# Lucaskabela/UNAST

Hardware: AMD Instinct MI355X
Metric: mel-frames/sec/node (train step, gen+disc) at B=32,T_mel=800; 1/2/4/8-GPU scaling (higher is better)
Workload: dtype bf16x3

## Files before the change

unast_amd/csrc/loss.hip:

```cpp
#include "common.h"

__global__ __launch_bounds__(256) void speech_loss_fwd_kernel(const float* __restrict__ gold, const float* __restrict__ head, int ldh,
                                                              const float* __restrict__ post, const int* __restrict__ lens, int B, int T, int M,
                                                              float eos_weight, double* __restrict__ ws, float* __restrict__ loss) {
    const int rows = B * T;
    const int mq = M >> 2;
    const size_t total = (size_t)rows * mq;
    float a0 = 0.f, a1 = 0.f, a2 = 0.f;
    for (size_t i = (size_t)blockIdx.x * 256 + threadIdx.x; i < total; i += (size_t)gridDim.x * 256) {
        const int r = (int)(i / mq), c = (int)(i - (size_t)r * mq) * 4;
        const int b = r / T, t = r - b * T;
        const int len = lens[b];
        if (t < len) {
            float4 g = *reinterpret_cast<const float4*>(gold + (size_t)r * M + c);
            float4 p = *reinterpret_cast<const float4*>(head + (size_t)r * ldh + c);
            float4 q = *reinterpret_cast<const float4*>(post + (size_t)r * M + c);
            float d;
            d = g.x - p.x; a0 += d * d; d = g.y - p.y; a0 += d * d; d = g.z - p.z; a0 += d * d; d = g.w - p.w; a0 += d * d;
            d = g.x - q.x; a1 += d * d; d = g.y - q.y; a1 += d * d; d = g.z - q.z; a1 += d * d; d = g.w - q.w; a1 += d * d;
        }
        if (c == 0) {
            const float x = head[(size_t)r * ldh + M];
            const float y = (t == len - 1) ? 1.f : 0.f;
            const float lw = 1.f + (eos_weight - 1.f) * y;
// ... 309 lines not shown
                    const float bb[4] = {b4.x, b4.y, b4.z, b4.w};
                    float gd[4] = {0.f, 0.f, 0.f, 0.f};
                    if (live) { const float4 g4 = *reinterpret_cast<const float4*>(gold + (size_t)m * M + n0); gd[0] = g4.x; gd[1] = g4.y; gd[2] = g4.z; gd[3] = g4.w; }
#pragma unroll
                    for (int r = 0; r < 4; ++r) {
                        const float p = acc[c2][r] + bb[r];
                        hp[r] = p;
                        if (live) { const float d = p - gd[r]; a0 += d * d; dp[r] = km * d; }
                    }
                } else if (n0 == M) {
                    const float x = acc[c2][0] + bias[M];
                    const float y = (tt == len - 1) ? 1.f : 0.f;
                    const float lw = 1.f + (eos_weight - 1.f) * y;
                    hp[0] = x;
                    a2 += (1.f - y) * x + lw * (log1pf(expf(-fabsf(x))) + fmaxf(-x, 0.f));
                    dp[0] = ks * ((1.f - y) - lw * (1.f - 1.f / (1.f + expf(-x))));
                }
                *reinterpret_cast<float4*>(head + (size_t)m * ldh + n0) = hv;
                *reinterpret_cast<float4*>(d_head + (size_t)m * ldh + n0) = dv;
            }
        }
    }
    __shared__ double red[8][2];
    const double d0 = wave_sum_d((double)a0), d2 = wave_sum_d((double)a2);
    if (lane == 0) { red[wave][0] = d0; red[wave][1] = d2; }
    __syncthreads();
    if (t < 2) {
        double v = 0.0;
        for (int w = 0; w < 8; ++w) v += red[w][t];
        atomicAdd(ws + (t == 0 ? 0 : 2), v);
    }
}

__global__ __launch_bounds__(256) void speech_post_loss_kernel(const float* __restrict__ gold, const float* __restrict__ post, const int* __restrict__ lens,
                                                               int B, int T, int M, float gscale, float* __restrict__ d_post, double* __restrict__ ws,
                                                               float* __restrict__ loss) {
    __shared__ float s_denom;
    if (threadIdx.x == 0) {
        double sl = 0.0;
        for (int b = 0; b < B; ++b) sl += (double)lens[b];
        s_denom = (float)(sl * (double)M);
    }
    __syncthreads();
    const float km = 2.f * gscale / s_denom;
    const int rows = B * T, mq = M >> 2;
    const size_t total = (size_t)rows * mq;
    float a1 = 0.f;
    for (size_t i = (size_t)blockIdx.x * 256 + threadIdx.x; i < total; i += (size_t)gridDim.x * 256) {
        const int r = (int)(i / mq), c = (int)(i - (size_t)r * mq) * 4;
        const int b = r / T, t = r - b * T;
        float4 o = make_float4(0.f, 0.f, 0.f, 0.f);
        if (t < lens[b]) {
            const float4 g = *reinterpret_cast<const float4*>(gold + (size_t)r * M + c);
            const float4 q = *reinterpret_cast<const float4*>(post + (size_t)r * M + c);
            const float dx = q.x - g.x, dy = q.y - g.y, dz = q.z - g.z, dw = q.w - g.w;
            a1 += (dx * dx + dy * dy) + (dz * dz + dw * dw);
            o = make_float4(km * dx, km * dy, km * dz, km * dw);
        }
        *reinterpret_cast<float4*>(d_post + (size_t)r * M + c) = o;
    }
    __shared__ double red[4];
    const double d1 = wave_sum_d((double)a1);
    if ((threadIdx.x & 63) == 0) red[threadIdx.x >> 6] = d1;
    __syncthreads();
    if (threadIdx.x == 0) {
        atomicAdd(ws + 1, (red[0] + red[1]) + (red[2] + red[3]));
        __threadfence();
        const unsigned long long arrived = atomicAdd(reinterpret_cast<unsigned long long*>(ws + 3), 1ull) + 1ull;
        if (arrived == gridDim.x) {
            __threadfence();
            const double s0 = atomicAdd(ws + 0, 0.0), s1 = atomicAdd(ws + 1, 0.0), s2 = atomicAdd(ws + 2, 0.0);
            const double denom = (double)s_denom;
            loss[0] = (float)(s0 / denom + s1 / denom + s2 / ((double)B * T));
            ws[0] = 0.0; ws[1] = 0.0; ws[2] = 0.0; reinterpret_cast<unsigned long long*>(ws)[3] = 0ull;
        }
    }
}

__global__ __launch_bounds__(256) void disc_targets_kernel(const int64_t* __restrict__ perm, int n, int B, int flip, float smoothing, float* __restrict__ out) {
    for (int i = threadIdx.x; i < n; i += 256) {
        float y = 1.f - smoothing;
        if (perm[i] >= B) y = 1.f - y;
        if (flip) y = 1.f - y;
        out[i] = y;
    }
}

__global__ __launch_bounds__(256) void bce_logits_kernel(const float* __restrict__ logits, int ldx, const float* __restrict__ targets, int n,
                                                         const float* __restrict__ gscale, float* __restrict__ loss, float* __restrict__ dlogits, int ldd) {
    __shared__ float red[4];
    float a = 0.f;
    const float g = gscale ? gscale[0] : 0.f;
    for (int i = threadIdx.x; i < n; i += 256) {
        const float y = targets[i];
        const float x = logits[(size_t)i * ldx];
// ... 129 lines not shown
    UNAST_REQUIRE(a && out && div != 0.f, "unast_scalar_combine: bad arguments");
    hipLaunchKernelGGL(scalar_combine_kernel, dim3(1), dim3(64), 0, stream, a, b, c, div, out);
    return unast_check_launch("unast_scalar_combine");
}

extern "C" int unast_text_head_loss(const float* X, int ldx, const float* W, const float* bias, const int64_t* gold, int rows, int K, int V,
                                    float eos_weight, float gscale, float* logits, float* dlogits, int ldl, double* ws, float* loss, hipStream_t stream) {
    const int eos_idx = 2, pad_idx = 0;
    UNAST_REQUIRE(X && W && bias && gold && logits && dlogits && ws && loss && rows > 0, "unast_text_head_loss: bad arguments");
    UNAST_REQUIRE(K == 256 && V > 0 && V <= 48 && ldl >= V && ldl <= 48 && (ldl & 3) == 0 && (ldx & 3) == 0, "unast_text_head_loss: built for K = 256, V <= 48, 16-byte row strides (K=%d V=%d ldl=%d)", K, V, ldl);
    UNAST_REQUIRE((((uintptr_t)X | (uintptr_t)W | (uintptr_t)logits | (uintptr_t)dlogits) & 15) == 0, "unast_text_head_loss: operands must be 16-byte aligned");
    hipLaunchKernelGGL(text_head_loss_kernel, dim3((rows + 127) / 128), dim3(512), 0, stream, X, ldx, W, bias, gold, rows, V, eos_idx, eos_weight, pad_idx,
                       gscale, logits, dlogits, ldl, ws, loss);
    return unast_check_launch("unast_text_head_loss");
}

extern "C" int unast_speech_head_loss(const float* X, int ldx, const float* W, const float* bias, const float* gold, const int* lens, int B, int T, int K, int M,
                                      float eos_weight, float gscale, float* head, float* d_head, int ldh, double* ws, hipStream_t stream) {
    UNAST_REQUIRE(X && W && bias && gold && lens && head && d_head && ws && B > 0 && T > 0, "unast_speech_head_loss: bad arguments");
    UNAST_REQUIRE(K == 256 && M > 0 && (M & 3) == 0 && M + 1 <= 96 && ldh >= M + 1 && ldh <= 96 && (ldh & 3) == 0 && (ldx & 3) == 0,
                  "unast_speech_head_loss: built for K = 256, M %% 4 == 0, M + 1 <= 96 (K=%d M=%d ldh=%d)", K, M, ldh);
    UNAST_REQUIRE((((uintptr_t)X | (uintptr_t)W | (uintptr_t)bias | (uintptr_t)gold | (uintptr_t)head | (uintptr_t)d_head) & 15) == 0, "unast_speech_head_loss: operands must be 16-byte aligned");
    static bool attr = [] { return hipFuncSetAttribute((const void*)speech_head_loss_kernel, hipFuncAttributeMaxDynamicSharedMemorySize, 2 * 96 * 512) == hipSuccess; }();
    (void)attr;
    const int rows = B * T;
    hipLaunchKernelGGL(speech_head_loss_kernel, dim3((rows + 127) / 128), dim3(512), 2 * 96 * 512, stream, X, ldx, W, bias, gold, lens, B, T, M, eos_weight, gscale,
                       head, d_head, ldh, ws);
    return unast_check_launch("unast_speech_head_loss");
}

extern "C" int unast_speech_post_loss(const float* gold, const float* post, const int* lens, int B, int T, int M, float gscale, float* d_post, double* ws,
                                      float* loss, hipStream_t stream) {
    UNAST_REQUIRE(gold && post && lens && d_post && ws && loss && B > 0 && T > 0 && M > 0 && (M & 3) == 0, "unast_speech_post_loss: bad arguments");
    hipLaunchKernelGGL(speech_post_loss_kernel, dim3(ls_grid((size_t)B * T * (M / 4))), dim3(256), 0, stream, gold, post, lens, B, T, M, gscale, d_post, ws, loss);
    return unast_check_launch("unast_speech_post_loss");
}

UNAST_DEFINE_RNG_EPOCH_SETTER(loss)
```

unast_amd/csrc/norm.hip:

```cpp
#include "common.h"

#define LN_MAXV 4
__global__ __launch_bounds__(256) void layernorm_fwd_kernel(const float* __restrict__ z, const float* __restrict__ gamma,
                                                            const float* __restrict__ beta, float* __restrict__ y,
                                                            float* __restrict__ mean, float* __restrict__ rstd,
                                                            int rows, int C, float eps) {
    const int lane = threadIdx.x & 63;
    const int row = blockIdx.x * 4 + (threadIdx.x >> 6);
    if (row >= rows) return;
    const float* zr = z + (size_t)row * C;
    float4 v[LN_MAXV];
    float s = 0.f;
#pragma unroll
    for (int i = 0; i < LN_MAXV; ++i) {
        int c = (lane + 64 * i) * 4;
        if (c < C) {
            v[i] = *reinterpret_cast<const float4*>(zr + c);
            s += (v[i].x + v[i].y) + (v[i].z + v[i].w);
        }
    }
    const float mu = wave_sum(s) / (float)C;
    float q = 0.f;
#pragma unroll
    for (int i = 0; i < LN_MAXV; ++i) {
// ... 167 lines not shown
#pragma unroll
            for (int u = 0; u < 4; ++u) {
                a.x += v[u].x; a.y += v[u].y; a.z += v[u].z; a.w += v[u].w;
                q.x += v[u].x * v[u].x; q.y += v[u].y * v[u].y; q.z += v[u].z * v[u].z; q.w += v[u].w * v[u].w;
            }
        }
        for (; r < r1; r += nry) {
            float4 v = *reinterpret_cast<const float4*>(x + (size_t)r * ldx + tx * 4);
            a.x += v.x; a.y += v.y; a.z += v.z; a.w += v.w;
            q.x += v.x * v.x; q.y += v.y * v.y; q.z += v.z * v.z; q.w += v.w * v.w;
        }
    }
    *reinterpret_cast<float4*>(red[0][threadIdx.x]) = a;
    *reinterpret_cast<float4*>(red[1][threadIdx.x]) = q;
    __syncthreads();
    for (int c = threadIdx.x; c < C; c += 256) {
        const int qd = c >> 2, e = c & 3;
        float sa = 0.f, sq = 0.f;
        for (int yy = 0; yy < nry; ++yy) { sa += red[0][yy * cq + qd][e]; sq += red[1][yy * cq + qd][e]; }
        atomicAdd(s1 + c, (ACC)sa);
        if (s2) atomicAdd(s2 + c, (ACC)sq);
    }
}

__global__ __launch_bounds__(256) void colsum_scalar_kernel(const float* __restrict__ x, int ldx, int rows, int C, int rows_per_block, float* __restrict__ s1) {
    const int r0 = blockIdx.x * rows_per_block, r1 = min(rows, r0 + rows_per_block);
    for (int c = threadIdx.x; c < C; c += 256) {
        float a = 0.f;
        for (int r = r0; r < r1; ++r) a += x[(size_t)r * ldx + c];
        atomicAdd(s1 + c, a);
    }
}

__device__ __forceinline__ float act_fwd(float x, int act) { return act == 1 ? fmaxf(x, 0.f) : (act == 2 ? tanhf(x) : x); }

__global__ __launch_bounds__(256) void bn_apply_fwd_kernel(const float* __restrict__ x, const double* __restrict__ s1, const double* __restrict__ s2,
                                                           double n, float eps, float momentum, float* __restrict__ mean, float* __restrict__ rstd,
                                                           float* __restrict__ running_mean, float* __restrict__ running_var,
                                                           long long* __restrict__ num_batches_tracked, int stats_given,
                                                           const float* __restrict__ gamma, const float* __restrict__ beta, float* __restrict__ y, int rows, int C,
                                                           int act, uint32_t drop_thresh, float drop_scale, uint32_t seed, uint32_t stream) {
    const int cq = C >> 2;
    const size_t total = (size_t)rows * cq;
    const bool fixed = ((size_t)gridDim.x * 256) % (size_t)cq == 0;
    float m[4], rs[4];
    auto stats = [&](int c) {
        if (stats_given) {
#pragma unroll
            for (int e = 0; e < 4; ++e) { m[e] = mean[c + e]; rs[e] = rstd[c + e]; }
            return;
        }
#pragma unroll
        for (int e = 0; e < 4; ++e) {
            const double mu = s1[c + e] / n;
            double var = s2[c + e] / n - mu * mu;
            if (var < 0.0) var = 0.0;
            m[e] = (float)mu;
            rs[e] = (float)(1.0 / sqrt(var + (double)eps));
        }
    };
    const size_t i0 = (size_t)blockIdx.x * 256 + threadIdx.x;
    if (fixed) stats((int)(i0 % cq) * 4);
    if (!stats_given && blockIdx.x == 0) {
        for (int c = threadIdx.x; c < C; c += 256) {
            const double mu = s1[c] / n;
            double var = s2[c] / n - mu * mu;
            if (var < 0.0) var = 0.0;
            mean[c] = (float)mu;
            rstd[c] = (float)(1.0 / sqrt(var + (double)eps));
            if (running_mean) {
                running_mean[c] = (1.f - momentum) * running_mean[c] + momentum * (float)mu;
                const double unb = n > 1.0 ? var * n / (n - 1.0) : var;
                running_var[c] = (1.f - momentum) * running_var[c] + momentum * (float)unb;
            }
        }
        if (num_batches_tracked && threadIdx.x == 0) *num_batches_tracked += 1;
    }
    for (size_t i = i0; i < total; i += (size_t)gridDim.x * 256) {
        const int r = (int)(i / cq), c = (int)(i - (size_t)r * cq) * 4;
        if (!fixed) stats(c);
        float4 v = *reinterpret_cast<const float4*>(x + (size_t)r * C + c);
        float4 g = *reinterpret_cast<const float4*>(gamma + c), b = *reinterpret_cast<const float4*>(beta + c);
        float o[4] = {(v.x - m[0]) * rs[0] * g.x + b.x, (v.y - m[1]) * rs[1] * g.y + b.y, (v.z - m[2]) * rs[2] * g.z + b.z,
                      (v.w - m[3]) * rs[3] * g.w + b.w};
        uint32_t rkey = drop_thresh ? rng_row_key(seed, stream, (uint32_t)r) : 0u;
#pragma unroll
        for (int e = 0; e < 4; ++e) {
            float a = act_fwd(o[e], act);
            if (drop_thresh) a = rng_keep(rkey, c + e, drop_thresh) ? a * drop_scale : 0.f;
            o[e] = a;
        }
        *reinterpret_cast<float4*>(y + (size_t)r * C + c) = make_float4(o[0], o[1], o[2], o[3]);
    }
}

__global__ __launch_bounds__(256) void bn_bwd_reduce_kernel(float* __restrict__ dy, const float* __restrict__ x,
                                                            const float* __restrict__ mean, const float* __restrict__ rstd,
                                                            const float* __restrict__ gamma, const float* __restrict__ beta,
                                                            int rows, int C, int rows_per_block, int act, uint32_t drop_thresh,
                                                            float drop_scale, uint32_t seed, uint32_t stream,
                                                            double* __restrict__ S1, double* __restrict__ S2) {
    __shared__ float red[2][256][4];
    const int cq = C >> 2;
    const int nry = 256 / cq;
    const int tx = threadIdx.x % cq, ty = threadIdx.x / cq;
    const int c = tx * 4;
    float a[4] = {0, 0, 0, 0}, q[4] = {0, 0, 0, 0};
    const int r0 = blockIdx.x * rows_per_block, r1 = min(rows, r0 + rows_per_block);
    if (ty < nry) {
        float4 m = *reinterpret_cast<const float4*>(mean + c), s = *reinterpret_cast<const float4*>(rstd + c);
        float4 g = *reinterpret_cast<const float4*>(gamma + c), b = *reinterpret_cast<const float4*>(beta + c);
        const float mm[4] = {m.x, m.y, m.z, m.w}, ss[4] = {s.x, s.y, s.z, s.w}, gg[4] = {g.x, g.y, g.z, g.w}, bb[4] = {b.x, b.y, b.z, b.w};
        for (int r = r0 + ty; r < r1; r += nry) {
            float4 d4 = *reinterpret_cast<const float4*>(dy + (size_t)r * C + c);
            float4 x4 = *reinterpret_cast<const float4*>(x + (size_t)r * C + c);
            float d[4] = {d4.x, d4.y, d4.z, d4.w}, xv[4] = {x4.x, x4.y, x4.z, x4.w};
            uint32_t rkey = drop_thresh ? rng_row_key(seed, stream, (uint32_t)r) : 0u;
#pragma unroll
            for (int e = 0; e < 4; ++e) {
                const float xh = (xv[e] - mm[e]) * ss[e];
                const float pre = xh * gg[e] + bb[e];
                float dd = d[e];
                if (drop_thresh) dd = rng_keep(rkey, c + e, drop_thresh) ? dd * drop_scale : 0.f;
                if (act == 1) dd = pre > 0.f ? dd : 0.f;
                else if (act == 2) { const float th = tanhf(pre); dd *= (1.f - th * th); }
                d[e] = dd;
                a[e] += dd;
                q[e] += dd * xh;
            }
            *reinterpret_cast<float4*>(dy + (size_t)r * C + c) = make_float4(d[0], d[1], d[2], d[3]);
        }
    }
    *reinterpret_cast<float4*>(red[0][threadIdx.x]) = make_float4(a[0], a[1], a[2], a[3]);
    *reinterpret_cast<float4*>(red[1][threadIdx.x]) = make_float4(q[0], q[1], q[2], q[3]);
    __syncthreads();
    for (int cc = threadIdx.x; cc < C; cc += 256) {
        const int qd = cc >> 2, e = cc & 3;
        float sa = 0.f, sq = 0.f;
        for (int yy = 0; yy < nry; ++yy) { sa += red[0][yy * cq + qd][e]; sq += red[1][yy * cq + qd][e]; }
        atomicAdd(S1 + cc, (double)sa);
        atomicAdd(S2 + cc, (double)sq);
    }
}

__global__ __launch_bounds__(256) void bn_bwd_apply_kernel(const float* __restrict__ dpre, const float* __restrict__ x,
                                                           const float* __restrict__ mean, const float* __restrict__ rstd,
                                                           const float* __restrict__ gamma, const double* __restrict__ S1,
                                                           const double* __restrict__ S2, float* __restrict__ dx, int rows, int C,
                                                           float* __restrict__ dgamma, float* __restrict__ dbeta) {
    const int cq = C >> 2;
    const size_t total = (size_t)rows * cq;
    const float invn = 1.f / (float)rows;
    if (blockIdx.x == 0 && dgamma) {
        for (int c = threadIdx.x; c < C; c += 256) { dgamma[c] += (float)S2[c]; dbeta[c] += (float)S1[c]; }
    }
    for (size_t i = (size_t)blockIdx.x * 256 + threadIdx.x; i < total; i += (size_t)gridDim.x * 256) {
        const int r = (int)(i / cq), c = (int)(i - (size_t)r * cq) * 4;
        float4 d = *reinterpret_cast<const float4*>(dpre + (size_t)r * C + c);
        float4 xv = *reinterpret_cast<const float4*>(x + (size_t)r * C + c);
        float4 m = *reinterpret_cast<const float4*>(mean + c), s = *reinterpret_cast<const float4*>(rstd + c);
        float4 g = *reinterpret_cast<const float4*>(gamma + c);
        const float s1[4] = {(float)S1[c] * invn, (float)S1[c + 1] * invn, (float)S1[c + 2] * invn, (float)S1[c + 3] * invn};
        const float s2[4] = {(float)S2[c] * invn, (float)S2[c + 1] * invn, (float)S2[c + 2] * invn, (float)S2[c + 3] * invn};
// ... 38 lines not shown
                                   float drop_p, unsigned int seed, unsigned int stream_id, int finalize, hipStream_t stream) {
    UNAST_REQUIRE(dy && z && gamma && mean && rstd && dz, "unast_layernorm_bwd: null pointer");
    UNAST_REQUIRE((dgamma == nullptr) == (dbeta == nullptr), "unast_layernorm_bwd: dgamma/dbeta must both be given or both null");
    UNAST_REQUIRE(rows > 0 && (C & 3) == 0 && C <= 1024, "unast_layernorm_bwd: need C%%4==0, C<=1024 (C=%d)", C);
    int blocks, rpb;
    ln_bwd_geometry(rows, &blocks, &rpb);
    UNAST_REQUIRE(!dgamma || (ws && ws_floats >= (int64_t)blocks * 2 * C), "unast_layernorm_bwd: workspace too small (need %lld floats)", (long long)blocks * 2 * C);
    uint32_t th = dz_drop ? drop_threshold(drop_p) : 0u;
    float* const dzd = th ? dz_drop : (float*)nullptr;
    float* const prt = dgamma ? ws : (float*)nullptr;
    const float dsc = drop_p > 0.f ? 1.f / (1.f - drop_p) : 1.f;
    if (C <= 256)      hipLaunchKernelGGL((layernorm_bwd_kernel<1, 4>), dim3(blocks), dim3(256), 0, stream, dy, z, gamma, mean, rstd, dz, dzd, prt, rows, C, rpb, th, dsc, seed, stream_id);
    else if (C <= 512) hipLaunchKernelGGL((layernorm_bwd_kernel<2, 2>), dim3(blocks), dim3(256), 0, stream, dy, z, gamma, mean, rstd, dz, dzd, prt, rows, C, rpb, th, dsc, seed, stream_id);
    else               hipLaunchKernelGGL((layernorm_bwd_kernel<4, 1>), dim3(blocks), dim3(256), 0, stream, dy, z, gamma, mean, rstd, dz, dzd, prt, rows, C, rpb, th, dsc, seed, stream_id);
    if (dgamma && finalize) hipLaunchKernelGGL(ln_bwd_finalize_kernel, dim3((2 * C + 63) / 64), dim3(1024), 0, stream, ws, blocks, C, dgamma, dbeta);
    return unast_check_launch("unast_layernorm_bwd");
}

extern "C" int unast_layernorm_bwd_finalize(const float* ws, int64_t ws_floats, int rows, int C, float* dgamma, float* dbeta, hipStream_t stream) {
    UNAST_REQUIRE(ws && dgamma && dbeta && rows > 0 && (C & 3) == 0 && C <= 1024, "unast_layernorm_bwd_finalize: bad arguments");
    int blocks, rpb;
    ln_bwd_geometry(rows, &blocks, &rpb);
    UNAST_REQUIRE(ws_floats >= (int64_t)blocks * 2 * C, "unast_layernorm_bwd_finalize: workspace too small");
    hipLaunchKernelGGL(ln_bwd_finalize_kernel, dim3((2 * C + 63) / 64), dim3(1024), 0, stream, ws, blocks, C, dgamma, dbeta);
    return unast_check_launch("unast_layernorm_bwd_finalize");
}

extern "C" int unast_layernorm_partials_finalize(const float* part, int nblk, int C, float* dgamma, float* dbeta, hipStream_t stream) {
    UNAST_REQUIRE(part && dgamma && dbeta && nblk > 0 && C > 0 && C <= 1024, "unast_layernorm_partials_finalize: bad arguments");
    hipLaunchKernelGGL(ln_bwd_finalize_kernel, dim3((2 * C + 63) / 64), dim3(1024), 0, stream, part, nblk, C, dgamma, dbeta);
    return unast_check_launch("unast_layernorm_partials_finalize");
}

static int colsum_geometry(int rows, int C, int* blocks, int* rpb) {
    if ((C & 3) != 0 || C > 1024 || C <= 0) return -1;
    int b = grid_for(rows, 64, 1024);
    *rpb = (rows + b - 1) / b;
    *blocks = (rows + *rpb - 1) / *rpb;
    return 0;
}

__global__ __launch_bounds__(256) void colsum_det_part_kernel(const float* __restrict__ x, int ldx, int rows, int C, int rows_per_block, float* __restrict__ part) {
    const int r0 = blockIdx.x * rows_per_block, r1 = min(rows, r0 + rows_per_block);
    for (int c = threadIdx.x; c < C; c += 256) {
        float a = 0.f;
        for (int r = r0; r < r1; ++r) a += x[(size_t)r * ldx + c];
        part[(size_t)blockIdx.x * C + c] = a;
    }
}
__global__ __launch_bounds__(256) void colsum_det_final_kernel(const float* __restrict__ part, int blocks, int C, float* __restrict__ sum) {
    const int c = blockIdx.x * 256 + threadIdx.x;
    if (c >= C) return;
    float a = sum[c];
    for (int b = 0; b < blocks; ++b) a += part[(size_t)b * C + c];
    sum[c] = a;
}
static void colsum_det_geometry(int rows, int* blocks, int* rpb) {
    int b = grid_for(rows, 64, 512);
    *rpb = (rows + b - 1) / b;
    *blocks = (rows + *rpb - 1) / *rpb;
}
extern "C" int64_t unast_colsum_det_ws_floats(int rows, int C) {
    int blocks, rpb;
    colsum_det_geometry(rows, &blocks, &rpb);
    return (int64_t)blocks * C;
}
extern "C" int unast_colsum_det(const float* x, int ldx, int rows, int C, float* sum, float* ws, int64_t ws_floats, hipStream_t stream) {
    UNAST_REQUIRE(x && sum && ws && rows > 0 && C > 0, "unast_colsum_det: bad arguments");
    int blocks, rpb;
    colsum_det_geometry(rows, &blocks, &rpb);
    UNAST_REQUIRE(ws_floats >= (int64_t)blocks * C, "unast_colsum_det: workspace too small (need %lld floats)", (long long)blocks * C);
    hipLaunchKernelGGL(colsum_det_part_kernel, dim3(blocks), dim3(256), 0, stream, x, ldx, rows, C, rpb, ws);
    hipLaunchKernelGGL(colsum_det_final_kernel, dim3((C + 255) / 256), dim3(256), 0, stream, ws, blocks, C, sum);
    return unast_check_launch("unast_colsum_det");
}

extern "C" int unast_colsum_f32(const float* x, int ldx, int rows, int C, float* sum, hipStream_t stream) {
    UNAST_REQUIRE(x && sum, "unast_colsum_f32: null pointer");
    int blocks, rpb;
    UNAST_REQUIRE(rows > 0 && C > 0 && C <= 1024, "unast_colsum_f32: need 0 < C <= 1024");
    if ((C & 3) != 0 || (ldx & 3) != 0 || (((uintptr_t)x) & 15) != 0) {
        blocks = grid_for(rows, 64, 1024);
        rpb = (rows + blocks - 1) / blocks;
        blocks = (rows + rpb - 1) / rpb;
        hipLaunchKernelGGL(colsum_scalar_kernel, dim3(blocks), dim3(256), 0, stream, x, ldx, rows, C, rpb, sum);
        return unast_check_launch("unast_colsum_f32");
    }
    colsum_geometry(rows, C, &blocks, &rpb);
    hipLaunchKernelGGL((colsum_kernel<float>), dim3(blocks), dim3(256), 0, stream, x, ldx, rows, C, rpb, sum, (float*)nullptr);
    return unast_check_launch("unast_colsum_f32");
}

extern "C" int unast_bn_fwd(const float* x, const float* gamma, const float* beta, float* y, float* mean, float* rstd,
                            float* running_mean, float* running_var, double* ws , int rows, int C,
                            float eps, float momentum, int act, float drop_p, unsigned int seed, unsigned int stream_id,
                            int have_sums, int64_t* num_batches_tracked, hipStream_t stream) {
    UNAST_REQUIRE(x && gamma && beta && y && mean && rstd && ws, "unast_bn_fwd: null pointer");
    int blocks, rpb;
    UNAST_REQUIRE(colsum_geometry(rows, C, &blocks, &rpb) == 0, "unast_bn_fwd: need C%%4==0, C<=1024 (C=%d)", C);
    if (!have_sums) {
        hipMemsetAsync(ws, 0, sizeof(double) * 2 * C, stream);
        hipLaunchKernelGGL((colsum_kernel<double>), dim3(blocks), dim3(256), 0, stream, x, C, rows, C, rpb, ws, ws + C);
    }
    hipLaunchKernelGGL(bn_apply_fwd_kernel, dim3(grid_for((size_t)rows * (C / 4), 256)), dim3(256), 0, stream, x, ws, ws + C, (double)rows, eps, momentum,
                       mean, rstd, running_mean, running_var, (long long*)num_batches_tracked, 0, gamma, beta, y,
                       rows, C, act, drop_threshold(drop_p), drop_p > 0.f ? 1.f / (1.f - drop_p) : 1.f, seed, stream_id);
    return unast_check_launch("unast_bn_fwd");
}

__global__ void bn_eval_stats_kernel(const float* __restrict__ running_mean, const float* __restrict__ running_var, int C, float eps,
                                     float* __restrict__ mean, float* __restrict__ rstd) {
    const int c = blockIdx.x * blockDim.x + threadIdx.x;
    if (c >= C) return;
    mean[c] = running_mean[c];
    rstd[c] = 1.f / sqrtf(running_var[c] + eps);
}

extern "C" int unast_bn_eval_fwd(const float* x, const float* gamma, const float* beta, const float* running_mean,
                                 const float* running_var, float* y, float* mean, float* rstd, int rows, int C, float eps, int act,
                                 hipStream_t stream) {
    UNAST_REQUIRE(x && gamma && beta && running_mean && running_var && y && mean && rstd, "unast_bn_eval_fwd: null pointer");
    UNAST_REQUIRE(rows > 0 && C > 0 && C % 4 == 0, "unast_bn_eval_fwd: need rows>0, C%%4==0 (rows=%d C=%d)", rows, C);
    hipLaunchKernelGGL(bn_eval_stats_kernel, dim3((C + 255) / 256), dim3(256), 0, stream, running_mean, running_var, C, eps, mean, rstd);
    hipLaunchKernelGGL(bn_apply_fwd_kernel, dim3(grid_for((size_t)rows * (C / 4), 256)), dim3(256), 0, stream, x, (const double*)nullptr, (const double*)nullptr, 1.0, eps,
                       0.f, mean, rstd, (float*)nullptr, (float*)nullptr, (long long*)nullptr, 1, gamma, beta, y, rows, C, act, 0u, 1.f, 0u, 0u);
    return unast_check_launch("unast_bn_eval_fwd");
}

extern "C" int unast_bn_bwd(float* dy_inout, const float* x, const float* mean, const float* rstd, const float* gamma, const float* beta,
                            float* dx, float* dgamma, float* dbeta, double* ws , int rows, int C, int act,
                            float drop_p, unsigned int seed, unsigned int stream_id, int ws_zeroed, hipStream_t stream) {
    UNAST_REQUIRE(dy_inout && x && mean && rstd && gamma && beta && dx && ws, "unast_bn_bwd: null pointer");
    UNAST_REQUIRE((dgamma == nullptr) == (dbeta == nullptr), "unast_bn_bwd: dgamma/dbeta must both be given or both null");
    int blocks, rpb;
    UNAST_REQUIRE(colsum_geometry(rows, C, &blocks, &rpb) == 0, "unast_bn_bwd: need C%%4==0, C<=1024 (C=%d)", C);
    if (!ws_zeroed) hipMemsetAsync(ws, 0, sizeof(double) * 2 * C, stream);
    hipLaunchKernelGGL(bn_bwd_reduce_kernel, dim3(blocks), dim3(256), 0, stream, dy_inout, x, mean, rstd, gamma, beta, rows, C, rpb, act,
                       drop_threshold(drop_p), drop_p > 0.f ? 1.f / (1.f - drop_p) : 1.f, seed, stream_id, ws, ws + C);
    hipLaunchKernelGGL(bn_bwd_apply_kernel, dim3(grid_for((size_t)rows * (C / 4), 256)), dim3(256), 0, stream, dy_inout, x, mean, rstd, gamma,
                       ws, ws + C, dx, rows, C, dgamma, dbeta);
    return unast_check_launch("unast_bn_bwd");
}

UNAST_DEFINE_RNG_EPOCH_SETTER(norm)
```

unast_amd/csrc/optim.hip:

```cpp
#include "common.h"

__global__ __launch_bounds__(256) void sumsq_kernel(const float* __restrict__ g, size_t n4, size_t n, double* __restrict__ out) {
    float a = 0.f;
    double acc = 0.0;
    int cnt = 0;
    for (size_t i = (size_t)blockIdx.x * 256 + threadIdx.x; i < n4; i += (size_t)gridDim.x * 256) {
        float4 v = reinterpret_cast<const float4*>(g)[i];
        a += (v.x * v.x + v.y * v.y) + (v.z * v.z + v.w * v.w);
        if (++cnt == 64) { acc += (double)a; a = 0.f; cnt = 0; }
    }
    if (blockIdx.x == 0)
        for (size_t i = n4 * 4 + threadIdx.x; i < n; i += 256) a += g[i] * g[i];
    acc += (double)a;
    acc = wave_sum_d(acc);
    if ((threadIdx.x & 63) == 0) atomicAdd(out, acc);
}

__global__ __launch_bounds__(256) void adamw_kernel(float* __restrict__ p, float* __restrict__ g, float* __restrict__ m, float* __restrict__ v,
                                                    size_t n4, size_t n, const double* __restrict__ sumsq, float max_norm, float lr, float b1, float b2,
                                                    float eps, float wd, float bc1, float bc2_sqrt, float* __restrict__ split_out,
                                                    int decoupled, const float* __restrict__ dev_hyper, int zero_grad) {
    if (dev_hyper) { lr = dev_hyper[0]; bc1 = dev_hyper[1]; bc2_sqrt = dev_hyper[2]; }
    float coef = 1.f;
    if (max_norm > 0.f) {
        const float total = (float)sqrt(sumsq[0]);
        coef = fminf(max_norm / (total + 1e-6f), 1.f);
    }
    const float decay = decoupled ? 1.f - lr * wd : 1.f;
    const float l2 = decoupled ? 0.f : wd;
    const float step = lr / bc1;
    auto upd = [&](float& pp, float gg, float& mm, float& vv) {
        gg = gg * coef + l2 * pp;
        pp *= decay;
        mm = mm + (gg - mm) * (1.f - b1);
        vv = vv * b2 + (1.f - b2) * gg * gg;
        const float denom = sqrtf(vv) / bc2_sqrt + eps;
        pp = pp - step * (mm / denom);
    };
    for (size_t i = (size_t)blockIdx.x * 256 + threadIdx.x; i < n4; i += (size_t)gridDim.x * 256) {
        float4 P = reinterpret_cast<float4*>(p)[i], M = reinterpret_cast<float4*>(m)[i], V = reinterpret_cast<float4*>(v)[i];
        const float4 G = reinterpret_cast<const float4*>(g)[i];
        upd(P.x, G.x, M.x, V.x); upd(P.y, G.y, M.y, V.y); upd(P.z, G.z, M.z, V.z); upd(P.w, G.w, M.w, V.w);
        reinterpret_cast<float4*>(p)[i] = P; reinterpret_cast<float4*>(m)[i] = M; reinterpret_cast<float4*>(v)[i] = V;
        if (split_out) reinterpret_cast<uint4*>(split_out)[i] = split_chunk(P);
        if (zero_grad) reinterpret_cast<float4*>(g)[i] = make_float4(0.f, 0.f, 0.f, 0.f);
    }
    if (blockIdx.x == 0)
        for (size_t i = n4 * 4 + threadIdx.x; i < n; i += 256) {
            float pp = p[i], mm = m[i], vv = v[i];
            upd(pp, g[i], mm, vv);
            p[i] = pp; m[i] = mm; v[i] = vv;
            if (zero_grad) g[i] = 0.f;
        }
}

__global__ __launch_bounds__(256) void split_f32_kernel(const float* __restrict__ src, float* __restrict__ dst, size_t n4) {
    for (size_t i = (size_t)blockIdx.x * 256 + threadIdx.x; i < n4; i += (size_t)gridDim.x * 256)
        reinterpret_cast<uint4*>(dst)[i] = split_chunk(reinterpret_cast<const float4*>(src)[i]);
}

extern "C" int unast_sumsq(const float* g, int64_t n, double* out, hipStream_t stream) {
    UNAST_REQUIRE(g && out && n > 0, "unast_sumsq: bad arguments");
    UNAST_REQUIRE((((uintptr_t)g) & 15) == 0, "unast_sumsq: buffer must be 16-byte aligned");
    size_t blocks = ((size_t)n / 4 + 255) / 256;
    if (blocks < 1) blocks = 1;
    if (blocks > 1024) blocks = 1024;
    hipLaunchKernelGGL(sumsq_kernel, dim3((unsigned)blocks), dim3(256), 0, stream, g, (size_t)n / 4, (size_t)n, out);
    return unast_check_launch("unast_sumsq");
}

extern "C" int unast_adamw(float* p, float* g, float* m, float* v, int64_t n, const double* sumsq, float max_norm, float lr,
                           float beta1, float beta2, float eps, float weight_decay, int step, float* split_out, int decoupled,
                           const float* dev_hyper, int zero_grad, hipStream_t stream) {
    UNAST_REQUIRE(p && g && m && v && n > 0 && (step >= 1 || dev_hyper), "unast_adamw: bad arguments");
    if (step < 1) step = 1;
    UNAST_REQUIRE(!(max_norm > 0.f) || sumsq, "unast_adamw: clipping needs the sum-of-squares scalar");
    UNAST_REQUIRE(((((uintptr_t)p) | ((uintptr_t)g) | ((uintptr_t)m) | ((uintptr_t)v)) & 15) == 0, "unast_adamw: buffers must be 16-byte aligned");
    UNAST_REQUIRE(!split_out || ((((uintptr_t)split_out) & 15) == 0 && (n & 3) == 0), "unast_adamw: split_out needs 16-byte alignment and n %% 4 == 0");
    const double bc1 = 1.0 - pow((double)beta1, (double)step);
    const double bc2 = 1.0 - pow((double)beta2, (double)step);
    size_t blocks = ((size_t)n / 4 + 255) / 256;
    if (blocks < 1) blocks = 1;
    if (blocks > 4096) blocks = 4096;
    hipLaunchKernelGGL(adamw_kernel, dim3((unsigned)blocks), dim3(256), 0, stream, p, g, m, v, (size_t)n / 4, (size_t)n, sumsq, max_norm, lr, beta1,
                       beta2, eps, weight_decay, (float)bc1, (float)sqrt(bc2), split_out, decoupled, dev_hyper, zero_grad);
    return unast_check_launch("unast_adamw");
}

struct StepWords { unsigned int w[16]; };
__global__ __launch_bounds__(64) void set_words_kernel(unsigned int* __restrict__ dst, StepWords v, int n) {
    const int i = threadIdx.x;
    if (i < n) dst[i] = v.w[i];
}

extern "C" int unast_set_words(unsigned int* dst, const unsigned int* host_words, int n, hipStream_t stream) {
    UNAST_REQUIRE(dst && host_words && n > 0 && n <= 16, "unast_set_words: need 1..16 words");
    StepWords v;
    for (int i = 0; i < 16; ++i) v.w[i] = i < n ? host_words[i] : 0u;
    hipLaunchKernelGGL(set_words_kernel, dim3(1), dim3(64), 0, stream, dst, v, n);
// ... 44 lines not shown
```

Before: 950,300.

## Unroll loads in-flight across post-loss, batchnorm and sumsq kernels with templated variants

The speech post-loss, sumsq and batchnorm apply/backward-reduce kernels now keep several independent float4 loads in flight per thread through manual unrolling, and use fewer, larger blocks. Batchnorm kernels are templated on activation and dropout, so runtime branches become compile-time ones, and the forward apply switches to a row-block geometry where per-column stats are computed once per thread. Sumsq reduces within the block before one atomic per block, and post-loss redirects dead-row loads to a valid address instead of branching. The risks are higher register pressure from the unrolling and possibly less parallelism from the capped grids.

```diff
diff --git a/unast_amd/csrc/loss.hip b/unast_amd/csrc/loss.hip
--- a/unast_amd/csrc/loss.hip
+++ b/unast_amd/csrc/loss.hip
@@ -365,35 +365,59 @@
     }
 }
 
+#define POST_LOSS_U 8
+#define POST_LOSS_MAX_BLOCKS 512
 __global__ __launch_bounds__(256) void speech_post_loss_kernel(const float* __restrict__ gold, const float* __restrict__ post, const int* __restrict__ lens,
                                                                int B, int T, int M, float gscale, float* __restrict__ d_post, double* __restrict__ ws,
                                                                float* __restrict__ loss) {
+    constexpr int U = POST_LOSS_U;
     __shared__ float s_denom;
-    if (threadIdx.x == 0) {
-        double sl = 0.0;
-        for (int b = 0; b < B; ++b) sl += (double)lens[b];
-        s_denom = (float)(sl * (double)M);
-    }
-    __syncthreads();
+    __shared__ double red[4];
+    {
+        long long sl = 0;
+        for (int b = threadIdx.x; b < B; b += 256) sl += (long long)lens[b];
+#pragma unroll
+        for (int o = 32; o > 0; o >>= 1) sl += __shfl_xor(sl, o, 64);
+        if ((threadIdx.x & 63) == 0) red[threadIdx.x >> 6] = (double)sl;
+        __syncthreads();
+        if (threadIdx.x == 0) s_denom = (float)(((red[0] + red[1]) + (red[2] + red[3])) * (double)M);
+        __syncthreads();
+    }
     const float km = 2.f * gscale / s_denom;
     const int rows = B * T, mq = M >> 2;
-    const size_t total = (size_t)rows * mq;
-    float a1 = 0.f;
-    for (size_t i = (size_t)blockIdx.x * 256 + threadIdx.x; i < total; i += (size_t)gridDim.x * 256) {
-        const int r = (int)(i / mq), c = (int)(i - (size_t)r * mq) * 4;
-        const int b = r / T, t = r - b * T;
-        float4 o = make_float4(0.f, 0.f, 0.f, 0.f);
-        if (t < lens[b]) {
-            const float4 g = *reinterpret_cast<const float4*>(gold + (size_t)r * M + c);
-            const float4 q = *reinterpret_cast<const float4*>(post + (size_t)r * M + c);
-            const float dx = q.x - g.x, dy = q.y - g.y, dz = q.z - g.z, dw = q.w - g.w;
-            a1 += (dx * dx + dy * dy) + (dz * dz + dw * dw);
-            o = make_float4(km * dx, km * dy, km * dz, km * dw);
-        }
-        *reinterpret_cast<float4*>(d_post + (size_t)r * M + c) = o;
-    }
-    __shared__ double red[4];
-    const double d1 = wave_sum_d((double)a1);
+    const size_t total = (size_t)rows * mq, stride = (size_t)gridDim.x * 256;
+    double a1 = 0.0;
+    const size_t first = (size_t)blockIdx.x * 256 + threadIdx.x;
+    auto is_live = [&](size_t i) {
+        const uint32_t r = (uint32_t)i / (uint32_t)mq;
+        const uint32_t b = r / (uint32_t)T;
+        return (int)(r - b * (uint32_t)T) < lens[b];
+    };
+    auto group = [&](size_t i, bool live, const float4& g, const float4& q) {
+        const float dx = q.x - g.x, dy = q.y - g.y, dz = q.z - g.z, dw = q.w - g.w;
+        *reinterpret_cast<float4*>(d_post + i * 4) = live ? make_float4(km * dx, km * dy, km * dz, km * dw) : make_float4(0.f, 0.f, 0.f, 0.f);
+        return live ? (dx * dx + dy * dy) + (dz * dz + dw * dw) : 0.f;
+    };
+    size_t i = first;
+    for (; i + (U - 1) * stride < total; i += U * stride) {
+        float4 g[U], q[U];
+        bool live[U];
+#pragma unroll
+        for (int u = 0; u < U; ++u) {
+            live[u] = is_live(i + u * stride);
+            const size_t off = (live[u] ? i + u * stride : first) * 4;
+            g[u] = *reinterpret_cast<const float4*>(gold + off);
+            q[u] = *reinterpret_cast<const float4*>(post + off);
+        }
+#pragma unroll
+        for (int u = 0; u < U; ++u) a1 += (double)group(i + u * stride, live[u], g[u], q[u]);
+    }
+    for (; i < total; i += stride) {
+        const bool live = is_live(i);
+        const size_t off = (live ? i : first) * 4;
+        a1 += (double)group(i, live, *reinterpret_cast<const float4*>(gold + off), *reinterpret_cast<const float4*>(post + off));
+    }
+    const double d1 = wave_sum_d(a1);
     if ((threadIdx.x & 63) == 0) red[threadIdx.x >> 6] = d1;
     __syncthreads();
     if (threadIdx.x == 0) {
@@ -589,7 +613,9 @@
 extern "C" int unast_speech_post_loss(const float* gold, const float* post, const int* lens, int B, int T, int M, float gscale, float* d_post, double* ws,
                                       float* loss, hipStream_t stream) {
     UNAST_REQUIRE(gold && post && lens && d_post && ws && loss && B > 0 && T > 0 && M > 0 && (M & 3) == 0, "unast_speech_post_loss: bad arguments");
-    hipLaunchKernelGGL(speech_post_loss_kernel, dim3(ls_grid((size_t)B * T * (M / 4))), dim3(256), 0, stream, gold, post, lens, B, T, M, gscale, d_post, ws, loss);
+    UNAST_REQUIRE((size_t)B * T * (M / 4) < ((size_t)1 << 31), "unast_speech_post_loss: B * T * M / 4 must stay below 2^31");
+    const size_t per_block = (size_t)256 * POST_LOSS_U;
+    hipLaunchKernelGGL(speech_post_loss_kernel, dim3(ls_grid(((size_t)B * T * (M / 4) + per_block - 1) / per_block * 256, POST_LOSS_MAX_BLOCKS)), dim3(256), 0, stream, gold, post, lens, B, T, M, gscale, d_post, ws, loss);
     return unast_check_launch("unast_speech_post_loss");
 }
 
diff --git a/unast_amd/csrc/norm.hip b/unast_amd/csrc/norm.hip
--- a/unast_amd/csrc/norm.hip
+++ b/unast_amd/csrc/norm.hip
@@ -223,35 +223,25 @@
     }
 }
 
-__device__ __forceinline__ float act_fwd(float x, int act) { return act == 1 ? fmaxf(x, 0.f) : (act == 2 ? tanhf(x) : x); }
-
+#define BN_ROWS_IN_FLIGHT 4
+
+__device__ __forceinline__ void rng_keep4(uint32_t row_key, int c, uint32_t thresh, bool keep[4]) {
+    const uint32_t h0 = rng_pair(row_key, (uint32_t)c), h1 = rng_pair(row_key, (uint32_t)c + 2u);
+    keep[0] = rng_keep_lo(h0, thresh); keep[1] = rng_keep_hi(h0, thresh);
+    keep[2] = rng_keep_lo(h1, thresh); keep[3] = rng_keep_hi(h1, thresh);
+}
+
+template <int ACT, bool DROP>
 __global__ __launch_bounds__(256) void bn_apply_fwd_kernel(const float* __restrict__ x, const double* __restrict__ s1, const double* __restrict__ s2,
                                                            double n, float eps, float momentum, float* __restrict__ mean, float* __restrict__ rstd,
                                                            float* __restrict__ running_mean, float* __restrict__ running_var,
                                                            long long* __restrict__ num_batches_tracked, int stats_given,
                                                            const float* __restrict__ gamma, const float* __restrict__ beta, float* __restrict__ y, int rows, int C,
-                                                           int act, uint32_t drop_thresh, float drop_scale, uint32_t seed, uint32_t stream) {
-    const int cq = C >> 2;
-    const size_t total = (size_t)rows * cq;
-    const bool fixed = ((size_t)gridDim.x * 256) % (size_t)cq == 0;
-    float m[4], rs[4];
-    auto stats = [&](int c) {
-        if (stats_given) {
-#pragma unroll
-            for (int e = 0; e < 4; ++e) { m[e] = mean[c + e]; rs[e] = rstd[c + e]; }
-            return;
-        }
-#pragma unroll
-        for (int e = 0; e < 4; ++e) {
-            const double mu = s1[c + e] / n;
-            double var = s2[c + e] / n - mu * mu;
-            if (var < 0.0) var = 0.0;
-            m[e] = (float)mu;
-            rs[e] = (float)(1.0 / sqrt(var + (double)eps));
-        }
-    };
-    const size_t i0 = (size_t)blockIdx.x * 256 + threadIdx.x;
-    if (fixed) stats((int)(i0 % cq) * 4);
+                                                           int rows_per_block, uint32_t drop_thresh, float drop_scale, uint32_t seed, uint32_t stream) {
+    constexpr int RU = BN_ROWS_IN_FLIGHT;
+    const int cq = C >> 2, cw = min(cq, 256);
+    const int nry = 256 / cw;
+    const int tx = threadIdx.x % cw, ty = threadIdx.x / cw;
     if (!stats_given && blockIdx.x == 0) {
         for (int c = threadIdx.x; c < C; c += 256) {
             const double mu = s1[c] / n;
@@ -267,30 +257,59 @@
         }
         if (num_batches_tracked && threadIdx.x == 0) *num_batches_tracked += 1;
     }
-    for (size_t i = i0; i < total; i += (size_t)gridDim.x * 256) {
-        const int r = (int)(i / cq), c = (int)(i - (size_t)r * cq) * 4;
-        if (!fixed) stats(c);
-        float4 v = *reinterpret_cast<const float4*>(x + (size_t)r * C + c);
-        float4 g = *reinterpret_cast<const float4*>(gamma + c), b = *reinterpret_cast<const float4*>(beta + c);
-        float o[4] = {(v.x - m[0]) * rs[0] * g.x + b.x, (v.y - m[1]) * rs[1] * g.y + b.y, (v.z - m[2]) * rs[2] * g.z + b.z,
-                      (v.w - m[3]) * rs[3] * g.w + b.w};
-        uint32_t rkey = drop_thresh ? rng_row_key(seed, stream, (uint32_t)r) : 0u;
-#pragma unroll
-        for (int e = 0; e < 4; ++e) {
-            float a = act_fwd(o[e], act);
-            if (drop_thresh) a = rng_keep(rkey, c + e, drop_thresh) ? a * drop_scale : 0.f;
-            o[e] = a;
-        }
-        *reinterpret_cast<float4*>(y + (size_t)r * C + c) = make_float4(o[0], o[1], o[2], o[3]);
-    }
-}
-
+    if (ty >= nry) return;
+    const int r0 = blockIdx.x * rows_per_block, r1 = min(rows, r0 + rows_per_block);
+    const uint32_t rbase = DROP ? rng_stream_base(seed, stream) : 0u;
+    for (int qd = tx; qd < cq; qd += cw) {
+        const int c = qd * 4;
+        float m[4], rs[4];
+        if (stats_given) {
+#pragma unroll
+            for (int e = 0; e < 4; ++e) { m[e] = mean[c + e]; rs[e] = rstd[c + e]; }
+        } else {
+#pragma unroll
+            for (int e = 0; e < 4; ++e) {
+                const double mu = s1[c + e] / n;
+                double var = s2[c + e] / n - mu * mu;
+                if (var < 0.0) var = 0.0;
+                m[e] = (float)mu;
+                rs[e] = (float)(1.0 / sqrt(var + (double)eps));
+            }
+        }
+        const float4 g = *reinterpret_cast<const float4*>(gamma + c), b = *reinterpret_cast<const float4*>(beta + c);
+        auto row = [&](int r, const float4& v) {
+            float o[4] = {(v.x - m[0]) * rs[0] * g.x + b.x, (v.y - m[1]) * rs[1] * g.y + b.y, (v.z - m[2]) * rs[2] * g.z + b.z,
+                          (v.w - m[3]) * rs[3] * g.w + b.w};
+#pragma unroll
+            for (int e = 0; e < 4; ++e) o[e] = ACT == 1 ? fmaxf(o[e], 0.f) : (ACT == 2 ? tanhf(o[e]) : o[e]);
+            if (DROP) {
+                bool keep[4];
+                rng_keep4(pcg_hash((uint32_t)r + rbase), c, drop_thresh, keep);
+#pragma unroll
+                for (int e = 0; e < 4; ++e) o[e] = keep[e] ? o[e] * drop_scale : 0.f;
+            }
+            *reinterpret_cast<float4*>(y + (size_t)r * C + c) = make_float4(o[0], o[1], o[2], o[3]);
+        };
+        int r = r0 + ty;
+        for (; r + (RU - 1) * nry < r1; r += RU * nry) {
+            float4 v[RU];
+#pragma unroll
+            for (int u = 0; u < RU; ++u) v[u] = *reinterpret_cast<const float4*>(x + (size_t)(r + u * nry) * C + c);
+#pragma unroll
+            for (int u = 0; u < RU; ++u) row(r + u * nry, v[u]);
+        }
+        for (; r < r1; r += nry) row(r, *reinterpret_cast<const float4*>(x + (size_t)r * C + c));
+    }
+}
+
+template <int ACT, bool DROP>
 __global__ __launch_bounds__(256) void bn_bwd_reduce_kernel(float* __restrict__ dy, const float* __restrict__ x,
                                                             const float* __restrict__ mean, const float* __restrict__ rstd,
                                                             const float* __restrict__ gamma, const float* __restrict__ beta,
-                                                            int rows, int C, int rows_per_block, int act, uint32_t drop_thresh,
+                                                            int rows, int C, int rows_per_block, uint32_t drop_thresh,
                                                             float drop_scale, uint32_t seed, uint32_t stream,
                                                             double* __restrict__ S1, double* __restrict__ S2) {
+    constexpr int RU = BN_ROWS_IN_FLIGHT;
     __shared__ float red[2][256][4];
     const int cq = C >> 2;
     const int nry = 256 / cq;
@@ -302,24 +321,41 @@
         float4 m = *reinterpret_cast<const float4*>(mean + c), s = *reinterpret_cast<const float4*>(rstd + c);
         float4 g = *reinterpret_cast<const float4*>(gamma + c), b = *reinterpret_cast<const float4*>(beta + c);
         const float mm[4] = {m.x, m.y, m.z, m.w}, ss[4] = {s.x, s.y, s.z, s.w}, gg[4] = {g.x, g.y, g.z, g.w}, bb[4] = {b.x, b.y, b.z, b.w};
-        for (int r = r0 + ty; r < r1; r += nry) {
-            float4 d4 = *reinterpret_cast<const float4*>(dy + (size_t)r * C + c);
-            float4 x4 = *reinterpret_cast<const float4*>(x + (size_t)r * C + c);
-            float d[4] = {d4.x, d4.y, d4.z, d4.w}, xv[4] = {x4.x, x4.y, x4.z, x4.w};
-            uint32_t rkey = drop_thresh ? rng_row_key(seed, stream, (uint32_t)r) : 0u;
+        const uint32_t rbase = DROP ? rng_stream_base(seed, stream) : 0u;
+        auto row = [&](int r, const float4& d4, const float4& x4) {
+            float d[4] = {d4.x, d4.y, d4.z, d4.w};
+            const float xv[4] = {x4.x, x4.y, x4.z, x4.w};
+            bool keep[4] = {true, true, true, true};
+            if (DROP) rng_keep4(pcg_hash((uint32_t)r + rbase), c, drop_thresh, keep);
 #pragma unroll
             for (int e = 0; e < 4; ++e) {
                 const float xh = (xv[e] - mm[e]) * ss[e];
                 const float pre = xh * gg[e] + bb[e];
                 float dd = d[e];
-                if (drop_thresh) dd = rng_keep(rkey, c + e, drop_thresh) ? dd * drop_scale : 0.f;
-                if (act == 1) dd = pre > 0.f ? dd : 0.f;
-                else if (act == 2) { const float th = tanhf(pre); dd *= (1.f - th * th); }
+                if (DROP) dd = keep[e] ? dd * drop_scale : 0.f;
+                if (ACT == 1) dd = pre > 0.f ? dd : 0.f;
+                else if (ACT == 2) { const float th = tanhf(pre); dd *= (1.f - th * th); }
                 d[e] = dd;
                 a[e] += dd;
                 q[e] += dd * xh;
             }
             *reinterpret_cast<float4*>(dy + (size_t)r * C + c) = make_float4(d[0], d[1], d[2], d[3]);
+        };
+        int r = r0 + ty;
+        for (; r + (RU - 1) * nry < r1; r += RU * nry) {
+            float4 d4[RU], x4[RU];
+#pragma unroll
+            for (int u = 0; u < RU; ++u) {
+                const size_t off = (size_t)(r + u * nry) * C + c;
+                d4[u] = *reinterpret_cast<const float4*>(dy + off);
+                x4[u] = *reinterpret_cast<const float4*>(x + off);
+            }
+#pragma unroll
+            for (int u = 0; u < RU; ++u) row(r + u * nry, d4[u], x4[u]);
+        }
+        for (; r < r1; r += nry) {
+            const size_t off = (size_t)r * C + c;
+            row(r, *reinterpret_cast<const float4*>(dy + off), *reinterpret_cast<const float4*>(x + off));
         }
     }
     *reinterpret_cast<float4*>(red[0][threadIdx.x]) = make_float4(a[0], a[1], a[2], a[3]);
@@ -424,6 +460,14 @@
     return unast_check_launch("unast_layernorm_partials_finalize");
 }
 
+static void bn_fwd_geometry(int rows, int cw, int* blocks, int* rpb) {
+    const int step = BN_ROWS_IN_FLIGHT * (256 / cw);
+    int per = (rows + 1023) / 1024;
+    per = (per + step - 1) / step * step;
+    *rpb = per;
+    *blocks = (rows + per - 1) / per;
+}
+
 static int colsum_geometry(int rows, int C, int* blocks, int* rpb) {
     if ((C & 3) != 0 || C > 1024 || C <= 0) return -1;
     int b = grid_for(rows, 64, 1024);
@@ -483,6 +527,15 @@
     return unast_check_launch("unast_colsum_f32");
 }
 
+static decltype(&bn_apply_fwd_kernel<0, false>) bn_apply_fwd_variant(int act, bool drop) {
+    if (drop) return act == 1 ? bn_apply_fwd_kernel<1, true> : (act == 2 ? bn_apply_fwd_kernel<2, true> : bn_apply_fwd_kernel<0, true>);
+    return act == 1 ? bn_apply_fwd_kernel<1, false> : (act == 2 ? bn_apply_fwd_kernel<2, false> : bn_apply_fwd_kernel<0, false>);
+}
+static decltype(&bn_bwd_reduce_kernel<0, false>) bn_bwd_reduce_variant(int act, bool drop) {
+    if (drop) return act == 1 ? bn_bwd_reduce_kernel<1, true> : (act == 2 ? bn_bwd_reduce_kernel<2, true> : bn_bwd_reduce_kernel<0, true>);
+    return act == 1 ? bn_bwd_reduce_kernel<1, false> : (act == 2 ? bn_bwd_reduce_kernel<2, false> : bn_bwd_reduce_kernel<0, false>);
+}
+
 extern "C" int unast_bn_fwd(const float* x, const float* gamma, const float* beta, float* y, float* mean, float* rstd,
                             float* running_mean, float* running_var, double* ws , int rows, int C,
                             float eps, float momentum, int act, float drop_p, unsigned int seed, unsigned int stream_id,
@@ -494,9 +547,11 @@
         hipMemsetAsync(ws, 0, sizeof(double) * 2 * C, stream);
         hipLaunchKernelGGL((colsum_kernel<double>), dim3(blocks), dim3(256), 0, stream, x, C, rows, C, rpb, ws, ws + C);
     }
-    hipLaunchKernelGGL(bn_apply_fwd_kernel, dim3(grid_for((size_t)rows * (C / 4), 256)), dim3(256), 0, stream, x, ws, ws + C, (double)rows, eps, momentum,
+    const uint32_t th = drop_threshold(drop_p);
+    bn_fwd_geometry(rows, C >> 2, &blocks, &rpb);
+    hipLaunchKernelGGL(bn_apply_fwd_variant(act, th != 0u), dim3(blocks), dim3(256), 0, stream, x, ws, ws + C, (double)rows, eps, momentum,
                        mean, rstd, running_mean, running_var, (long long*)num_batches_tracked, 0, gamma, beta, y,
-                       rows, C, act, drop_threshold(drop_p), drop_p > 0.f ? 1.f / (1.f - drop_p) : 1.f, seed, stream_id);
+                       rows, C, rpb, th, drop_p > 0.f ? 1.f / (1.f - drop_p) : 1.f, seed, stream_id);
     return unast_check_launch("unast_bn_fwd");
 }
 
@@ -514,8 +569,10 @@
     UNAST_REQUIRE(x && gamma && beta && running_mean && running_var && y && mean && rstd, "unast_bn_eval_fwd: null pointer");
     UNAST_REQUIRE(rows > 0 && C > 0 && C % 4 == 0, "unast_bn_eval_fwd: need rows>0, C%%4==0 (rows=%d C=%d)", rows, C);
     hipLaunchKernelGGL(bn_eval_stats_kernel, dim3((C + 255) / 256), dim3(256), 0, stream, running_mean, running_var, C, eps, mean, rstd);
-    hipLaunchKernelGGL(bn_apply_fwd_kernel, dim3(grid_for((size_t)rows * (C / 4), 256)), dim3(256), 0, stream, x, (const double*)nullptr, (const double*)nullptr, 1.0, eps,
-                       0.f, mean, rstd, (float*)nullptr, (float*)nullptr, (long long*)nullptr, 1, gamma, beta, y, rows, C, act, 0u, 1.f, 0u, 0u);
+    int blocks, rpb;
+    bn_fwd_geometry(rows, C / 4 < 256 ? C / 4 : 256, &blocks, &rpb);
+    hipLaunchKernelGGL(bn_apply_fwd_variant(act, false), dim3(blocks), dim3(256), 0, stream, x, (const double*)nullptr, (const double*)nullptr, 1.0, eps,
+                       0.f, mean, rstd, (float*)nullptr, (float*)nullptr, (long long*)nullptr, 1, gamma, beta, y, rows, C, rpb, 0u, 1.f, 0u, 0u);
     return unast_check_launch("unast_bn_eval_fwd");
 }
 
@@ -527,8 +584,9 @@
     int blocks, rpb;
     UNAST_REQUIRE(colsum_geometry(rows, C, &blocks, &rpb) == 0, "unast_bn_bwd: need C%%4==0, C<=1024 (C=%d)", C);
     if (!ws_zeroed) hipMemsetAsync(ws, 0, sizeof(double) * 2 * C, stream);
-    hipLaunchKernelGGL(bn_bwd_reduce_kernel, dim3(blocks), dim3(256), 0, stream, dy_inout, x, mean, rstd, gamma, beta, rows, C, rpb, act,
-                       drop_threshold(drop_p), drop_p > 0.f ? 1.f / (1.f - drop_p) : 1.f, seed, stream_id, ws, ws + C);
+    const uint32_t th = drop_threshold(drop_p);
+    hipLaunchKernelGGL(bn_bwd_reduce_variant(act, th != 0u), dim3(blocks), dim3(256), 0, stream, dy_inout, x, mean, rstd, gamma, beta, rows, C, rpb,
+                       th, drop_p > 0.f ? 1.f / (1.f - drop_p) : 1.f, seed, stream_id, ws, ws + C);
     hipLaunchKernelGGL(bn_bwd_apply_kernel, dim3(grid_for((size_t)rows * (C / 4), 256)), dim3(256), 0, stream, dy_inout, x, mean, rstd, gamma,
                        ws, ws + C, dx, rows, C, dgamma, dbeta);
     return unast_check_launch("unast_bn_bwd");
diff --git a/unast_amd/csrc/optim.hip b/unast_amd/csrc/optim.hip
--- a/unast_amd/csrc/optim.hip
+++ b/unast_amd/csrc/optim.hip
@@ -1,19 +1,31 @@
 #include "common.h"
 
+#define SUMSQ_MAX_BLOCKS 256
+#define SUMSQ_U 8
 __global__ __launch_bounds__(256) void sumsq_kernel(const float* __restrict__ g, size_t n4, size_t n, double* __restrict__ out) {
-    float a = 0.f;
+    constexpr int U = SUMSQ_U;
+    __shared__ double red[4];
+    const size_t stride = (size_t)gridDim.x * 256;
     double acc = 0.0;
-    int cnt = 0;
-    for (size_t i = (size_t)blockIdx.x * 256 + threadIdx.x; i < n4; i += (size_t)gridDim.x * 256) {
-        float4 v = reinterpret_cast<const float4*>(g)[i];
-        a += (v.x * v.x + v.y * v.y) + (v.z * v.z + v.w * v.w);
-        if (++cnt == 64) { acc += (double)a; a = 0.f; cnt = 0; }
+    auto add = [&](const float4& v) { acc += (double)((v.x * v.x + v.y * v.y) + (v.z * v.z + v.w * v.w)); };
+    size_t i = (size_t)blockIdx.x * 256 + threadIdx.x;
+    for (; i + (U - 1) * stride < n4; i += U * stride) {
+        float4 v[U];
+#pragma unroll
+        for (int u = 0; u < U; ++u) v[u] = reinterpret_cast<const float4*>(g)[i + u * stride];
+#pragma unroll
+        for (int u = 0; u < U; ++u) add(v[u]);
     }
-    if (blockIdx.x == 0)
-        for (size_t i = n4 * 4 + threadIdx.x; i < n; i += 256) a += g[i] * g[i];
-    acc += (double)a;
+    for (; i < n4; i += stride) add(reinterpret_cast<const float4*>(g)[i]);
+    if (blockIdx.x == 0) {
+        float a = 0.f;
+        for (size_t j = n4 * 4 + threadIdx.x; j < n; j += 256) a += g[j] * g[j];
+        acc += (double)a;
+    }
     acc = wave_sum_d(acc);
-    if ((threadIdx.x & 63) == 0) atomicAdd(out, acc);
+    if ((threadIdx.x & 63) == 0) red[threadIdx.x >> 6] = acc;
+    __syncthreads();
+    if (threadIdx.x == 0) atomicAdd(out, (red[0] + red[1]) + (red[2] + red[3]));
 }
 
 __global__ __launch_bounds__(256) void adamw_kernel(float* __restrict__ p, float* __restrict__ g, float* __restrict__ m, float* __restrict__ v,
@@ -62,9 +74,9 @@
 extern "C" int unast_sumsq(const float* g, int64_t n, double* out, hipStream_t stream) {
     UNAST_REQUIRE(g && out && n > 0, "unast_sumsq: bad arguments");
     UNAST_REQUIRE((((uintptr_t)g) & 15) == 0, "unast_sumsq: buffer must be 16-byte aligned");
-    size_t blocks = ((size_t)n / 4 + 255) / 256;
+    size_t blocks = ((size_t)n / 4 + 256 * SUMSQ_U - 1) / (256 * SUMSQ_U);
     if (blocks < 1) blocks = 1;
-    if (blocks > 1024) blocks = 1024;
+    if (blocks > SUMSQ_MAX_BLOCKS) blocks = SUMSQ_MAX_BLOCKS;
     hipLaunchKernelGGL(sumsq_kernel, dim3((unsigned)blocks), dim3(256), 0, stream, g, (size_t)n / 4, (size_t)n, out);
     return unast_check_launch("unast_sumsq");
 }
```

Result: no change. 957,600 (median of 6 runs) (+0.8%).
